# wenbowen123/catgrasp

Hardware: NVIDIA H100
Metric: candidate grasps scored/sec (higher is better)
Workload: dtype f32 (128->1024 layer f16 x f16 single pass on wgmma, f32 accumulate; other layers bf16 hi/lo x3)

## Files before the change

### catgrasp_b200/csrc/cg_tc_ptx.cuh

```cuda
#pragma once
#include <cuda_bf16.h>
#include <cuda_fp16.h>
#include <stdint.h>

namespace cg_ptx {

__device__ __forceinline__ uint32_t smem_u32(const void *p) { return static_cast<uint32_t>(__cvta_generic_to_shared(p)); }
__device__ __forceinline__ void mbar_init(uint32_t bar, uint32_t count) {
  asm volatile("mbarrier.init.shared::cta.b64 [%0], %1;" ::"r"(bar), "r"(count));
}
__device__ __forceinline__ void mbar_init_fence() { asm volatile("fence.mbarrier_init.release.cluster;" ::: "memory"); }
__device__ __forceinline__ void mbar_expect_tx(uint32_t bar, uint32_t bytes) {
  asm volatile("mbarrier.arrive.expect_tx.shared::cta.b64 _, [%0], %1;" ::"r"(bar), "r"(bytes) : "memory");
}
__device__ __forceinline__ void mbar_arrive(uint32_t bar) {
  asm volatile("mbarrier.arrive.shared::cta.b64 _, [%0];" ::"r"(bar) : "memory");
}
__device__ __forceinline__ void mbar_wait(uint32_t bar, uint32_t parity) {
  asm volatile(
      "{\n\t.reg .pred p;\n\t"
      "CG_MBAR_WAIT:\n\t"
      "mbarrier.try_wait.parity.shared::cta.b64 p, [%0], %1;\n\t"
      "@!p bra CG_MBAR_WAIT;\n\t}"
      ::"r"(bar), "r"(parity)
      : "memory");
}
__device__ __forceinline__ void bulk_g2s(uint32_t dst, const void *src, uint32_t bytes, uint32_t bar) {
  asm volatile("cp.async.bulk.shared::cluster.global.mbarrier::complete_tx::bytes [%0], [%1], %2, [%3];" ::"r"(dst),
               "l"(src), "r"(bytes), "r"(bar)
               : "memory");
}
__device__ __forceinline__ void fence_proxy_async() { asm volatile("fence.proxy.async.shared::cta;" ::: "memory"); }

__device__ __forceinline__ uint64_t wg_desc(uint32_t saddr) {
  return (uint64_t)((saddr >> 4) & 0x3FFFu) | (1ull << 16) | ((uint64_t)(1024 >> 4) << 32) | (1ull << 62);
}
__device__ __forceinline__ void wg_fence() { asm volatile("wgmma.fence.sync.aligned;" ::: "memory"); }
__device__ __forceinline__ void wg_commit() { asm volatile("wgmma.commit_group.sync.aligned;" ::: "memory"); }
template <int N>
__device__ __forceinline__ void wg_wait() {
  asm volatile("wgmma.wait_group.sync.aligned %0;" ::"n"(N) : "memory");
}
template <int N>
__device__ __forceinline__ void wg_fence_regs(float *r) {
#pragma unroll
  for (int i = 0; i < N; i++) asm volatile("" : "+f"(r[i])::"memory");
}
template <int N>
__device__ __forceinline__ void wg_fence_regs(uint32_t *r) {
#pragma unroll
  for (int i = 0; i < N; i++) asm volatile("" : "+r"(r[i])::"memory");
}

#define CG_WG_D8(i) "+f"(d[i]), "+f"(d[i + 1]), "+f"(d[i + 2]), "+f"(d[i + 3]), "+f"(d[i + 4]), "+f"(d[i + 5]), \
                    "+f"(d[i + 6]), "+f"(d[i + 7])

template <bool F16>
__device__ __forceinline__ void wg_m64n64(float *d, const uint32_t *a, uint64_t bdesc, uint32_t accumulate) {
  if (F16) {
    asm volatile(
        "{\n\t.reg .pred p;\n\t"
        "setp.ne.b32 p, %37, 0;\n\t"
        "wgmma.mma_async.sync.aligned.m64n64k16.f32.f16.f16 "
        "{%0, %1, %2, %3, %4, %5, %6, %7, %8, %9, %10, %11, %12, %13, %14, %15, "
        "%16, %17, %18, %19, %20, %21, %22, %23, %24, %25, %26, %27, %28, %29, %30, %31}, "
        "{%32, %33, %34, %35}, %36, p, 1, 1, 0;\n\t}"
        : CG_WG_D8(0), CG_WG_D8(8), CG_WG_D8(16), CG_WG_D8(24)
        : "r"(a[0]), "r"(a[1]), "r"(a[2]), "r"(a[3]), "l"(bdesc), "r"(accumulate)
        : "memory");
  } else {
    asm volatile(
        "{\n\t.reg .pred p;\n\t"
        "setp.ne.b32 p, %37, 0;\n\t"
        "wgmma.mma_async.sync.aligned.m64n64k16.f32.bf16.bf16 "
        "{%0, %1, %2, %3, %4, %5, %6, %7, %8, %9, %10, %11, %12, %13, %14, %15, "
        "%16, %17, %18, %19, %20, %21, %22, %23, %24, %25, %26, %27, %28, %29, %30, %31}, "
        "{%32, %33, %34, %35}, %36, p, 1, 1, 0;\n\t}"
        : CG_WG_D8(0), CG_WG_D8(8), CG_WG_D8(16), CG_WG_D8(24)
        : "r"(a[0]), "r"(a[1]), "r"(a[2]), "r"(a[3]), "l"(bdesc), "r"(accumulate)
        : "memory");
  }
}

template <bool F16>
__device__ __forceinline__ void wg_m64n128(float *d, const uint32_t *a, uint64_t bdesc, uint32_t accumulate) {
  if (F16) {
    asm volatile(
        "{\n\t.reg .pred p;\n\t"
        "setp.ne.b32 p, %69, 0;\n\t"
        "wgmma.mma_async.sync.aligned.m64n128k16.f32.f16.f16 "
        "{%0, %1, %2, %3, %4, %5, %6, %7, %8, %9, %10, %11, %12, %13, %14, %15, "
        "%16, %17, %18, %19, %20, %21, %22, %23, %24, %25, %26, %27, %28, %29, %30, %31, "
        "%32, %33, %34, %35, %36, %37, %38, %39, %40, %41, %42, %43, %44, %45, %46, %47, "
        "%48, %49, %50, %51, %52, %53, %54, %55, %56, %57, %58, %59, %60, %61, %62, %63}, "
        "{%64, %65, %66, %67}, %68, p, 1, 1, 0;\n\t}"
        : CG_WG_D8(0), CG_WG_D8(8), CG_WG_D8(16), CG_WG_D8(24), CG_WG_D8(32), CG_WG_D8(40), CG_WG_D8(48), CG_WG_D8(56)
        : "r"(a[0]), "r"(a[1]), "r"(a[2]), "r"(a[3]), "l"(bdesc), "r"(accumulate)
        : "memory");
  } else {
    asm volatile(
        "{\n\t.reg .pred p;\n\t"
        "setp.ne.b32 p, %69, 0;\n\t"
        "wgmma.mma_async.sync.aligned.m64n128k16.f32.bf16.bf16 "
        "{%0, %1, %2, %3, %4, %5, %6, %7, %8, %9, %10, %11, %12, %13, %14, %15, "
        "%16, %17, %18, %19, %20, %21, %22, %23, %24, %25, %26, %27, %28, %29, %30, %31, "
        "%32, %33, %34, %35, %36, %37, %38, %39, %40, %41, %42, %43, %44, %45, %46, %47, "
        "%48, %49, %50, %51, %52, %53, %54, %55, %56, %57, %58, %59, %60, %61, %62, %63}, "
        "{%64, %65, %66, %67}, %68, p, 1, 1, 0;\n\t}"
        : CG_WG_D8(0), CG_WG_D8(8), CG_WG_D8(16), CG_WG_D8(24), CG_WG_D8(32), CG_WG_D8(40), CG_WG_D8(48), CG_WG_D8(56)
        : "r"(a[0]), "r"(a[1]), "r"(a[2]), "r"(a[3]), "l"(bdesc), "r"(accumulate)
        : "memory");
  }
}
#undef CG_WG_D8

__device__ __forceinline__ void split_bf16x2(float x0, float x1, uint32_t &h, uint32_t &l) {
  const __nv_bfloat162 hh = __floats2bfloat162_rn(x0, x1);
  h = *reinterpret_cast<const uint32_t *>(&hh);
  const __nv_bfloat162 ll = __floats2bfloat162_rn(x0 - __uint_as_float(h << 16), x1 - __uint_as_float(h & 0xffff0000u));
  l = *reinterpret_cast<const uint32_t *>(&ll);
}
__device__ __forceinline__ void split_f16x2(float x0, float x1, uint32_t &h, uint32_t &l) {
  x0 = fminf(fmaxf(x0, -65504.f), 65504.f);
  x1 = fminf(fmaxf(x1, -65504.f), 65504.f);
  const __half2 hh = __floats2half2_rn(x0, x1);
  const float2 hf = __half22float2(hh);
  const __half2 ll = __floats2half2_rn(x0 - hf.x, x1 - hf.y);
  h = *reinterpret_cast<const uint32_t *>(&hh);
  l = *reinterpret_cast<const uint32_t *>(&ll);
}

template <int KS, bool F16>
__device__ __forceinline__ void d_to_a(const float *d, uint32_t (*hi)[4], uint32_t (*lo)[4]) {
#pragma unroll
  for (int j = 0; j < KS; j++)
#pragma unroll
    for (int r = 0; r < 4; r++) {
      if (F16) split_f16x2(d[8 * j + 2 * r], d[8 * j + 2 * r + 1], hi[j][r], lo[j][r]);
      else split_bf16x2(d[8 * j + 2 * r], d[8 * j + 2 * r + 1], hi[j][r], lo[j][r]);
    }
}

__host__ __device__ __forceinline__ uint32_t row_chunk_off(int row, int c16) {
  return (uint32_t)(row >> 3) * 1024u + (uint32_t)(row & 7) * 128u + (uint32_t)((c16 ^ (row & 7)) << 4);
}

}
```

### catgrasp_b200/csrc/cg_trunk_tc.cu

```cuda
#include <limits.h>
#include <stdlib.h>

#include <algorithm>

#include "cg_tc_ptx.cuh"
#include "cg_trunk_common.cuh"

namespace {
using namespace cg_trunk;
using namespace cg_ptx;

constexpr int NCW = 8;
constexpr int PROD_WARP = NCW;
constexpr int HELP_WARP = NCW + 1;
constexpr int NHELP = 3 * 32;
constexpr int NTC = (NCW + 4) * 32;
constexpr int NCHUNK = 8;
constexpr uint32_t PIECE = 16384;
constexpr uint32_t W1_OFF = 0;
constexpr uint32_t W2_OFF = PIECE;
constexpr uint32_t RING_OFF = 3 * PIECE;
constexpr uint32_t RING_BYTES = 8 * PIECE;
constexpr uint32_t SACC_OFF = RING_OFF + RING_BYTES;
constexpr uint32_t SACC_BYTES = 2 * 2 * NCHUNK * 4 * 32 * 8;
constexpr uint32_t KEYS_OFF = SACC_OFF + SACC_BYTES;
constexpr uint32_t KEYS_BYTES = 2 * 1024 * 4;
constexpr uint32_t MISC_OFF = KEYS_OFF + KEYS_BYTES;
constexpr int NSLOT_MAX = 8;
constexpr uint32_t IMG_W3B = NCHUNK * 2 * 2 * PIECE;
constexpr uint32_t IMG_W2 = 2 * PIECE, IMG_W1 = PIECE;
constexpr uint32_t IMG_W2_OFF = IMG_W3B, IMG_W1_OFF = IMG_W3B + IMG_W2;
constexpr uint32_t IMG_W3H_OFF = IMG_W1_OFF + IMG_W1;
constexpr uint32_t IMG_W3H = NCHUNK * 2 * PIECE;

struct Misc {
  float w0[6 * 64];
  float bias0[64];
  float bias1[64];
  float bias2[128];
  double pinv[12];
  double mean[6];
  double sden[6];
  float T3[12];
  unsigned long long full_bar[NSLOT_MAX];
  unsigned long long empty_bar[NSLOT_MAX];
  unsigned long long w_bar;
  unsigned long long cand_bar;
  unsigned long long front_bar;
  unsigned long long keys_bar[2];
};

constexpr size_t SMEM_BYTES = MISC_OFF + sizeof(Misc);
static_assert(SMEM_BYTES <= 232448, "exceeds the 227 KB per-CTA shared memory of sm_90");

template <int STEP>
__device__ __forceinline__ void max_butterfly_step(float *x, int lane) {
  const bool up = (lane & STEP) != 0;
#pragma unroll
  for (int k = 0; k < STEP / 2; k++) {
    const float send = up ? x[k] : x[k + STEP / 2];
    const float keep = up ? x[k + STEP / 2] : x[k];
    x[k] = fmaxf(keep, __shfl_xor_sync(0xffffffffu, send, STEP));
  }
}

#ifdef CG_EXPERIMENTS
enum { TL_START, TL_INPUT, TL_FRONT, TL_L3, TL_L3_WAIT, TL_RING, TL_NPHASE };
constexpr int TL_CTAS = 8, TL_REC = 8;
__host__ __device__ constexpr int TL_STRIDE(int B) { return B >= TL_CTAS ? B / TL_CTAS : 1; }
#define TL_PARAM , unsigned long long *tl
#define TL_ARG(p) , p
#else
#define TL_PARAM
#define TL_ARG(p)
#endif

template <int PASSES>
__global__ void __launch_bounds__(NTC, 1) trunk_tc_kernel(const cg_trunk_args a TL_PARAM) {
  constexpr int NSLOT = PASSES == 3 ? 4 : 8;
  constexpr uint32_t SLOT_BYTES = PASSES == 3 ? 2 * PIECE : PIECE;
  constexpr bool F16 = PASSES < 3;
  extern __shared__ __align__(1024) unsigned char smem[];
  if ((smem_u32(smem) & 1023u) != 0u) __trap();
  Misc &S = *reinterpret_cast<Misc *>(smem + MISC_OFF);
  float2 *sacc = reinterpret_cast<float2 *>(smem + SACC_OFF);
  uint32_t *keys = reinterpret_cast<uint32_t *>(smem + KEYS_OFF);
  const int tid = threadIdx.x, warp = __shfl_sync(0xffffffffu, tid >> 5, 0), lane = tid & 31;
  const int N = a.N;
  const int ntiles = (N + TP - 1) / TP;
  const long long T = (long long)a.B * ntiles;
  const int t_begin = (int)(blockIdx.x * T / gridDim.x);
  const int my_tiles = (int)((blockIdx.x + 1) * T / gridDim.x) - t_begin;
  const int b_first = t_begin / ntiles;
  const int ncand = (t_begin + my_tiles - 1) / ntiles - b_first + 1;
  const unsigned char *img = static_cast<const unsigned char *>(a.tc_img);
  const bool has_l1 = a.stage1_mode != 0;
  const uint32_t smem_s = smem_u32(smem);
  const uint32_t w1_s = smem_s + W1_OFF, w2_s = smem_s + W2_OFF, ring_s = smem_s + RING_OFF;
  const uint32_t misc_s = smem_s + MISC_OFF;
  const uint32_t full_s = misc_s + (uint32_t)offsetof(Misc, full_bar), empty_s = misc_s + (uint32_t)offsetof(Misc, empty_bar);
  const uint32_t wbar_s = misc_s + (uint32_t)offsetof(Misc, w_bar);
  const uint32_t cand_s = misc_s + (uint32_t)offsetof(Misc, cand_bar), front_s = misc_s + (uint32_t)offsetof(Misc, front_bar);
  const uint32_t keys_s = misc_s + (uint32_t)offsetof(Misc, keys_bar);

  for (int i = tid; i < 6 * 64; i += NTC) S.w0[i] = a.l0.Wt[i];
  if (tid < 64) {
    S.bias0[tid] = a.l0.b[tid];
    S.bias1[tid] = (a.stage1_mode == 1) ? a.l1.b[tid] : 0.f;
  }
  if (tid < 128) S.bias2[tid] = a.l2.b[tid];
  if (a.in.x_direct == nullptr && tid < 6) {
    S.mean[tid] = a.in.mean ? a.in.mean[tid] : 0.0;
    S.sden[tid] = a.in.stdv ? 1.0 / (a.in.stdv[tid] + 1e-15) : 1.0;
  }
  for (int i = tid; i < (int)(SACC_BYTES / 8); i += NTC) sacc[i] = make_float2(-INFINITY, -INFINITY);
  for (int i = tid; i < 2 * 1024; i += NTC) keys[i] = 0u;
  if (tid == 0) {
    for (int i = 0; i < NSLOT; i++) {
      mbar_init(full_s + 8u * i, 1);
      mbar_init(empty_s + 8u * i, NCW);
    }
    mbar_init(wbar_s, 1);
    mbar_init(cand_s, NHELP);
    mbar_init(front_s, NCW * 32);
    mbar_init(keys_s, NCW * 32);
    mbar_init(keys_s + 8u, NCW * 32);
    mbar_init_fence();
  }
  __syncthreads();

  if (warp == PROD_WARP) {
    if (lane == 0) {
      mbar_expect_tx(wbar_s, IMG_W2 + (a.stage1_mode == 1 ? IMG_W1 : 0u));
      bulk_g2s(w2_s, img + IMG_W2_OFF, IMG_W2, wbar_s);
      if (a.stage1_mode == 1) bulk_g2s(w1_s, img + IMG_W1_OFF, IMG_W1, wbar_s);
      const unsigned char *w3src = img + (PASSES == 3 ? 0u : IMG_W3H_OFF);
      const int total = my_tiles * NCHUNK * 2;
      for (int gs = 0; gs < total; gs++) {
        const int s = gs % NSLOT;
        mbar_wait(empty_s + 8u * s, (((uint32_t)(gs / NSLOT)) & 1u) ^ 1u);
        mbar_expect_tx(full_s + 8u * s, SLOT_BYTES);
        bulk_g2s(ring_s + (uint32_t)s * SLOT_BYTES, w3src + (size_t)(gs % (NCHUNK * 2)) * SLOT_BYTES, SLOT_BYTES,
                 full_s + 8u * s);
      }
    }
    return;
  }

  if (warp >= HELP_WARP) {
    const int ht = tid - HELP_WARP * 32;
    for (int k = 0; k <= ncand; k++) {
      if (k < ncand) {
        const int b = b_first + k;
        constexpr int TU = (64 * 8 + NHELP - 1) / NHELP;
        uint32_t t64h[TU][4], t64l[TU][4];
        if (a.stage1_mode == 2) {
          const float *Tb = a.T64 + (size_t)b * 4096;
#pragma unroll
          for (int i = 0; i < TU; i++) {
            const int u = ht + NHELP * i;
            if (u < 512) {
              float v[8];
#pragma unroll
              for (int e = 0; e < 8; e++) v[e] = __ldg(Tb + (8 * (u >> 6) + e) * 64 + (u & 63));
#pragma unroll
              for (int e = 0; e < 4; e++) split_bf16x2(v[2 * e], v[2 * e + 1], t64h[i][e], t64l[i][e]);
            }
          }
        }
        double pinv[12];
        const bool do_pinv = a.in.x_direct == nullptr && ht == 0;
        if (do_pinv) pose_inverse(a.in.poses + (size_t)b * 16, pinv);
        const float t3 = (a.T3 && ht < 9) ? a.T3[b * 9 + ht] : 0.f;
        if (k > 0) mbar_wait(front_s, (uint32_t)(k - 1) & 1u);
        if (a.stage1_mode == 2) {
#pragma unroll
          for (int i = 0; i < TU; i++) {
            const int u = ht + NHELP * i;
            if (u < 512) {
              const uint32_t off = row_chunk_off(u & 63, u >> 6);
              *reinterpret_cast<uint4 *>(smem + W1_OFF + off) =
                  make_uint4(t64h[i][0], t64h[i][1], t64h[i][2], t64h[i][3]);
              *reinterpret_cast<uint4 *>(smem + W1_OFF + 8192 + off) =
                  make_uint4(t64l[i][0], t64l[i][1], t64l[i][2], t64l[i][3]);
            }
          }
          fence_proxy_async();
        }
        if (do_pinv) {
#pragma unroll
          for (int i = 0; i < 12; i++) S.pinv[i] = pinv[i];
        }
        if (ht < 9) S.T3[ht] = t3;
        mbar_arrive(cand_s);
      }
      if (k > 0) {
        const int kp = k - 1;
        mbar_wait(keys_s + 8u * (kp & 1), ((uint32_t)kp >> 1) & 1u);
        uint32_t *kb = keys + (kp & 1) * 1024;
        uint32_t *g = a.gmax_keys + (size_t)(b_first + kp) * 1024;
        for (int ch = ht; ch < 1024; ch += NHELP) {
          float m = cg_key2f(kb[ch]) + __ldg(&a.l3.b[ch]);
          if (a.relu3) m = fmaxf(m, 0.f);
          atomicMax(&g[ch], cg_f2key(m));
          kb[ch] = 0u;
        }
      }
    }
    return;
  }

  const int wg = warp >> 2, w4 = warp & 3, g = lane >> 2, q = lane & 3;
  float vmax = 0.f;
#ifdef CG_EXPERIMENTS
  const bool tl_on = tl != nullptr && blockIdx.x % TL_STRIDE(gridDim.x) == 0 &&
                     (int)(blockIdx.x / TL_STRIDE(gridDim.x)) < TL_CTAS;
  unsigned long long tl_sum[TL_NPHASE] = {}, tl_t0 = clock64(), tl_t = tl_t0, tl_s;
#define TL_MARK(phase)                   \
  do {                                   \
    const unsigned long long _t = clock64(); \
    tl_sum[phase] += _t - tl_t;          \
    tl_t = _t;                           \
  } while (0)
#define TL_SPAN_BEGIN() (tl_s = clock64())
#define TL_SPAN_END(phase) (tl_sum[phase] += clock64() - tl_s)
#else
#define TL_MARK(phase) ((void)0)
#define TL_SPAN_BEGIN() ((void)0)
#define TL_SPAN_END(phase) ((void)0)
#endif
  mbar_wait(wbar_s, 0u);

  auto fetch_id = [&](int b, int n) -> int {
    if (n >= N) n = N - 1;
    return (a.in.x_direct == nullptr && a.in.ids) ? __ldg(a.in.ids + (size_t)b * N + n) : n;
  };
  auto fetch_row = [&](int b, int id, double *r) {
    if (a.in.x_direct) {
      const float *xr = a.in.x_direct + ((size_t)b * N + id) * 6;
#pragma unroll
      for (int k = 0; k < 6; k++) r[k] = __ldg(xr + k);
    } else {
      const double *px = a.in.cloud_xyz + (size_t)id * 3;
      const double *pn = a.in.cloud_nrm + (size_t)id * 3;
#pragma unroll
      for (int k = 0; k < 3; k++) {
        r[k] = __ldg(px + k);
        r[3 + k] = __ldg(pn + k);
      }
    }
  };
  auto finish_row = [&](const double *r, float *v) {
    if (a.in.x_direct) {
#pragma unroll
      for (int k = 0; k < 6; k++) v[k] = (float)r[k];
    } else {
      const double x = r[0], y = r[1], z = r[2];
      const double nx = r[3], ny = r[4], nz = r[5];
      const double *R = S.pinv;
      double w[6];
      w[0] = R[0] * x + R[1] * y + R[2] * z + R[9];
      w[1] = R[3] * x + R[4] * y + R[5] * z + R[10];
      w[2] = R[6] * x + R[7] * y + R[8] * z + R[11];
      w[3] = R[0] * nx + R[1] * ny + R[2] * nz;
      w[4] = R[3] * nx + R[4] * ny + R[5] * nz;
      w[5] = R[6] * nx + R[7] * ny + R[8] * nz;
#pragma unroll
      for (int k = 0; k < 6; k++) v[k] = (float)((w[k] - S.mean[k]) * S.sden[k]);
    }
    if (a.T3) {
      const float x = v[0], y = v[1], z = v[2];
      v[0] = fmaf(z, S.T3[6], fmaf(y, S.T3[3], x * S.T3[0]));
      v[1] = fmaf(z, S.T3[7], fmaf(y, S.T3[4], x * S.T3[1]));
      v[2] = fmaf(z, S.T3[8], fmaf(y, S.T3[5], x * S.T3[2]));
    }
  };

  uint32_t gslot = 0;
  auto slot_of = [&](int c, int kb) { return (gslot + 2u * c + kb) % NSLOT; };
  auto phase_of = [&](int c, int kb) { return ((gslot + 2u * c + kb) / NSLOT) & 1u; };

  const int prow = wg * 64 + w4 * 16 + g;
  constexpr int L3_GROUP = PASSES == 1 ? 8 : 4;
  constexpr bool ROW_PREFETCH = PASSES == 1;
  double r0[6], r1[6];
  int id0, id1;
  {
    const int j = t_begin - b_first * ntiles;
    id0 = fetch_id(b_first, j * TP + prow);
    id1 = fetch_id(b_first, j * TP + prow + 8);
    if (ROW_PREFETCH) {
      fetch_row(b_first, id0, r0);
      fetch_row(b_first, id1, r1);
    }
  }
  if (wg == 1) asm volatile("bar.sync 2, 256;" ::: "memory");
  TL_MARK(TL_START);
  for (int it = 0; it < my_tiles; it++) {
    const int b = (t_begin + it) / ntiles, j = t_begin + it - b * ntiles, ci = b - b_first;
    const bool cand_first = it == 0 || j == 0, cand_last = it + 1 == my_tiles || j + 1 == ntiles;
    const int p0 = j * TP + prow;
    if (cand_first) mbar_wait(cand_s, (uint32_t)ci & 1u);
    float d64[32];
    {
      float v0[6], v1[6];
      if (!ROW_PREFETCH) {
        fetch_row(b, id0, r0);
        fetch_row(b, id1, r1);
      }
      finish_row(r0, v0);
      finish_row(r1, v1);
      TL_MARK(TL_INPUT);
#pragma unroll
      for (int m = 0; m < 8; m++)
#pragma unroll
        for (int e = 0; e < 2; e++) {
          const int c = 8 * m + 2 * q + e;
          float o0 = S.bias0[c], o1 = o0;
#pragma unroll
          for (int k = 0; k < 6; k++) {
            const float w = S.w0[k * 64 + c];
            o0 = fmaf(v0[k], w, o0);
            o1 = fmaf(v1[k], w, o1);
          }
          d64[4 * m + e] = fmaxf(o0, 0.f);
          d64[4 * m + 2 + e] = fmaxf(o1, 0.f);
        }
    }
    uint32_t xh[8][4], xl[8][4];
    if (has_l1) {
      d_to_a<4, false>(d64, xh, xl);
      wg_fence_regs<16>(xh[0]);
      wg_fence_regs<16>(xl[0]);
      wg_fence_regs<32>(d64);
      wg_fence();
#pragma unroll
      for (int ks = 0; ks < 4; ks++) {
        const uint64_t bh = wg_desc(w1_s + 32u * ks), bl = wg_desc(w1_s + 8192u + 32u * ks);
        wg_m64n64<false>(d64, xl[ks], bh, ks > 0 ? 1u : 0u);
        wg_m64n64<false>(d64, xh[ks], bl, 1u);
        wg_m64n64<false>(d64, xh[ks], bh, 1u);
      }
      wg_commit();
      wg_wait<0>();
      wg_fence_regs<32>(d64);
      wg_fence_regs<16>(xh[0]);
      wg_fence_regs<16>(xl[0]);
#pragma unroll
      for (int i = 0; i < 32; i++) {
        if (a.stage1_mode == 1) d64[i] = fmaxf(d64[i] + S.bias1[8 * (i >> 2) + 2 * q + (i & 1)], 0.f);
      }
      if (a.pf_out) {
#pragma unroll
        for (int r = 0; r < 2; r++) {
          const int n = p0 + 8 * r;
          if (n < N) {
            float *dst = a.pf_out + ((size_t)b * N + n) * 64 + 2 * q;
#pragma unroll
            for (int m = 0; m < 8; m++)
              *reinterpret_cast<float2 *>(dst + 8 * m) = make_float2(d64[4 * m + 2 * r], d64[4 * m + 2 * r + 1]);
          }
        }
      }
    }
    if (cand_last) mbar_arrive(front_s);
    float acc[64];
    d_to_a<4, false>(d64, xh, xl);
    wg_fence_regs<16>(xh[0]);
    wg_fence_regs<16>(xl[0]);
    wg_fence_regs<64>(acc);
    wg_fence();
#pragma unroll
    for (int ks = 0; ks < 4; ks++) {
      const uint64_t bh = wg_desc(w2_s + 32u * ks), bl = wg_desc(w2_s + PIECE + 32u * ks);
      wg_m64n128<false>(acc, xl[ks], bh, ks > 0 ? 1u : 0u);
      wg_m64n128<false>(acc, xh[ks], bl, 1u);
      wg_m64n128<false>(acc, xh[ks], bh, 1u);
    }
    wg_commit();
    wg_wait<0>();
    wg_fence_regs<64>(acc);
    wg_fence_regs<16>(xh[0]);
    wg_fence_regs<16>(xl[0]);
    if (it == 0 && wg == 0) asm volatile("bar.arrive 2, 256;" ::: "memory");
    TL_MARK(TL_FRONT);
#pragma unroll
    for (int i = 0; i < 64; i++) acc[i] = fmaxf(acc[i] + S.bias2[8 * (i >> 2) + 2 * q + (i & 1)], 0.f);
    if (PASSES == 1) {
#pragma unroll
      for (int j = 0; j < 8; j++)
#pragma unroll
        for (int r = 0; r < 4; r++) {
          const float x0 = acc[8 * j + 2 * r], x1 = acc[8 * j + 2 * r + 1];
          vmax = fmaxf(vmax, fmaxf(x0, x1));
          asm("cvt.rn.satfinite.f16x2.f32 %0, %1, %2;" : "=r"(xh[j][r]) : "f"(x1), "f"(x0));
        }
    } else {
      if (PASSES == 2) {
#pragma unroll
        for (int i = 0; i < 64; i++) vmax = fmaxf(vmax, acc[i]);
      }
      d_to_a<8, F16>(acc, xh, xl);
    }
    wg_fence_regs<32>(xh[0]);
    if (PASSES != 1) wg_fence_regs<32>(xl[0]);
    auto issue = [&](int h, float *d) {
      const int c = h >> 1;
      if ((h & 1) == 0) {
        TL_SPAN_BEGIN();
        mbar_wait(full_s + 8u * slot_of(c, 0), phase_of(c, 0));
        mbar_wait(full_s + 8u * slot_of(c, 1), phase_of(c, 1));
        TL_SPAN_END(TL_RING);
      }
      wg_fence_regs<32>(d);
      wg_fence();
#pragma unroll
      for (int kb = 0; kb < 2; kb++) {
        const uint32_t ws = ring_s + slot_of(c, kb) * SLOT_BYTES + (uint32_t)(h & 1) * (PIECE / 2);
#pragma unroll
        for (int ks = 0; ks < 4; ks++) {
          const int j = kb * 4 + ks;
          const uint32_t first = (kb | ks) ? 1u : 0u;
          const uint64_t bw = wg_desc(ws + 32u * ks);
          if (PASSES == 3) {
            const uint64_t bl = wg_desc(ws + PIECE + 32u * ks);
            wg_m64n64<false>(d, xl[j], bw, first);
            wg_m64n64<false>(d, xh[j], bl, 1u);
            wg_m64n64<false>(d, xh[j], bw, 1u);
          } else if (PASSES == 2) {
            wg_m64n64<true>(d, xl[j], bw, first);
            wg_m64n64<true>(d, xh[j], bw, 1u);
          } else {
            wg_m64n64<true>(d, xh[j], bw, first);
          }
        }
      }
      wg_commit();
      wg_fence_regs<32>(d);
    };
    auto reduce = [&](int h, const float *d) {
      const int c = h >> 1;
      if (h & 1) {
        __syncwarp();
        if (lane == 0) {
          mbar_arrive(empty_s + 8u * slot_of(c, 0));
          mbar_arrive(empty_s + 8u * slot_of(c, 1));
        }
      }
      float x[16];
#pragma unroll
      for (int i = 0; i < 8; i++) {
        x[2 * i] = fmaxf(d[4 * i], d[4 * i + 2]);
        x[2 * i + 1] = fmaxf(d[4 * i + 1], d[4 * i + 3]);
      }
      max_butterfly_step<16>(x, lane);
      max_butterfly_step<8>(x, lane);
      max_butterfly_step<4>(x, lane);
      float2 &slot = sacc[((wg * 2 * NCHUNK + h) * 4 + w4) * 32 + lane];
      const float2 old = slot;
      slot = make_float2(fmaxf(old.x, x[0]), fmaxf(old.y, x[1]));
    };
    const int nt = t_begin + it + (it + 1 < my_tiles ? 1 : 0);
    const int nb = nt / ntiles, pn = (nt - nb * ntiles) * TP + prow;
    id0 = fetch_id(nb, pn);
    id1 = fetch_id(nb, pn + 8);
#pragma unroll 1
    for (int h0 = 0; h0 < 2 * NCHUNK; h0 += L3_GROUP) {
      if (ROW_PREFETCH && h0 == L3_GROUP) {
        fetch_row(nb, id0, r0);
        fetch_row(nb, id1, r1);
      }
      float acc3[2][32];
      issue(h0, acc3[0]);
#pragma unroll
      for (int j = 0; j < L3_GROUP; j++) {
        if (j + 1 < L3_GROUP) issue(h0 + j + 1, acc3[(j + 1) & 1]);
        TL_SPAN_BEGIN();
        if (j + 1 < L3_GROUP) wg_wait<1>();
        else wg_wait<0>();
        TL_SPAN_END(TL_L3_WAIT);
        wg_fence_regs<32>(acc3[j & 1]);
        reduce(h0 + j, acc3[j & 1]);
      }
    }
    wg_fence_regs<32>(xh[0]);
    if (PASSES != 1) wg_fence_regs<32>(xl[0]);
    gslot += 2u * NCHUNK;
    if (cand_last) {
      uint32_t *kk = keys + (ci & 1) * 1024;
#pragma unroll 4
      for (int h = 0; h < 2 * NCHUNK; h++) {
        float2 &slot = sacc[((wg * 2 * NCHUNK + h) * 4 + w4) * 32 + lane];
        const float2 v = slot;
        atomicMax(&kk[64 * h + 2 * lane], cg_f2key(v.x));
        atomicMax(&kk[64 * h + 2 * lane + 1], cg_f2key(v.y));
        slot = make_float2(-INFINITY, -INFINITY);
      }
      mbar_arrive(keys_s + 8u * (ci & 1));
    }
    TL_MARK(TL_L3);
  }
  if (F16 && vmax > 65504.f && a.ovf_flag) atomicOr(a.ovf_flag, 1u);
#ifdef CG_EXPERIMENTS
  if (tl_on && lane == 0) {
    unsigned long long *o = tl + ((size_t)(blockIdx.x / TL_STRIDE(gridDim.x)) * NCW + warp) * TL_REC;
#pragma unroll
    for (int p = 0; p < TL_NPHASE; p++) o[p] = tl_sum[p];
    o[TL_NPHASE] = (unsigned long long)my_tiles;
    o[TL_NPHASE + 1] = clock64() - tl_t0;
  }
#endif
#undef TL_MARK
#undef TL_SPAN_BEGIN
#undef TL_SPAN_END
}

}

size_t cg_tc_image_bytes() { return (size_t)IMG_W3H_OFF + IMG_W3H; }

int cg_tc_prepare(cg_ctx *ctx, const float *Wt3, const float *Wt2, const float *Wt1, void *dst_dev, int *f16_ok) {
  CG_CUDA(ctx, cudaFuncSetAttribute(trunk_tc_kernel<3>, cudaFuncAttributeMaxDynamicSharedMemorySize, (int)SMEM_BYTES));
  CG_CUDA(ctx, cudaFuncSetAttribute(trunk_tc_kernel<2>, cudaFuncAttributeMaxDynamicSharedMemorySize, (int)SMEM_BYTES));
  CG_CUDA(ctx, cudaFuncSetAttribute(trunk_tc_kernel<1>, cudaFuncAttributeMaxDynamicSharedMemorySize, (int)SMEM_BYTES));
  float wmax = 0.f;
  for (size_t i = 0; i < (size_t)128 * 1024; i++) wmax = fmaxf(wmax, fabsf(Wt3[i]));
  *f16_ok = (wmax < 65504.f) ? 1 : 0;
  std::vector<unsigned char> img(cg_tc_image_bytes(), 0);
  for (int ch = 0; ch < NCHUNK; ch++)
    for (int kb = 0; kb < 2; kb++) {
      unsigned char *hi = img.data() + (size_t)(ch * 2 + kb) * 2 * PIECE;
      cg_pack_bf16x2_block(Wt3, 1024, ch * 128, 128, kb * 64, hi, hi + PIECE);
    }
  cg_pack_bf16x2_block(Wt2, 128, 0, 128, 0, img.data() + IMG_W2_OFF, img.data() + IMG_W2_OFF + PIECE);
  if (Wt1) cg_pack_bf16x2_block(Wt1, 64, 0, 64, 0, img.data() + IMG_W1_OFF, img.data() + IMG_W1_OFF + 8192);
  for (int ch = 0; ch < NCHUNK; ch++)
    for (int r = 0; r < 128; r++)
      for (int k = 0; k < 128; k++) {
        const __half h = __float2half_rn(Wt3[(size_t)k * 1024 + ch * 128 + r]);
        unsigned short bits;
        memcpy(&bits, &h, 2);
        const size_t off = (size_t)IMG_W3H_OFF + (size_t)(ch * 2 + (k >> 6)) * PIECE + row_chunk_off(r, (k & 63) >> 3) +
                           (size_t)(k & 7) * 2;
        memcpy(img.data() + off, &bits, 2);
      }
  CG_CUDA(ctx, cudaMemcpyAsync(dst_dev, img.data(), img.size(), cudaMemcpyHostToDevice, ctx->stream));
  CG_CUDA(ctx, cudaStreamSynchronize(ctx->stream));
  return CG_OK;
}

int cg_trunk_launch_tc(cg_ctx *ctx, const cg_trunk_args &a) {
  CG_REQUIRE(ctx, a.B > 0 && a.N > 0, "trunk: B,N must be positive");
  CG_REQUIRE(ctx, a.tc_img != nullptr, "trunk: tensor-core weight image missing");
  const long long tiles = (long long)a.B * ((a.N + TP - 1) / TP);
  CG_REQUIRE(ctx, tiles <= INT_MAX, "trunk: too many tiles in one launch");
  const int grid = (int)std::min<long long>(ctx->num_sms, tiles);
  const int passes = !a.tc_f16_ok || ctx->engine == 1 ? 3 : (ctx->engine == 2 ? 2 : 1);
#ifdef CG_EXPERIMENTS
  static const bool timeline = getenv("CG_TRUNK_TIMELINE") && atoi(getenv("CG_TRUNK_TIMELINE")) != 0;
  unsigned long long *tl = nullptr;
  const size_t tl_words = (size_t)TL_CTAS * NCW * TL_REC;
  if (timeline) {
    CG_CUDA(ctx, cudaMallocAsync(&tl, tl_words * 8, ctx->stream));
    CG_CUDA(ctx, cudaMemsetAsync(tl, 0, tl_words * 8, ctx->stream));
  }
#endif
  if (passes == 3) trunk_tc_kernel<3><<<grid, NTC, SMEM_BYTES, ctx->stream>>>(a TL_ARG(tl));
  else if (passes == 2) trunk_tc_kernel<2><<<grid, NTC, SMEM_BYTES, ctx->stream>>>(a TL_ARG(tl));
  else trunk_tc_kernel<1><<<grid, NTC, SMEM_BYTES, ctx->stream>>>(a TL_ARG(tl));
  CG_LAUNCH_CHECK(ctx);
#ifdef CG_EXPERIMENTS
  if (timeline) {
    std::vector<unsigned long long> h(tl_words);
    CG_CUDA(ctx, cudaMemcpyAsync(h.data(), tl, tl_words * 8, cudaMemcpyDeviceToHost, ctx->stream));
    CG_CUDA(ctx, cudaFreeAsync(tl, ctx->stream));
    CG_CUDA(ctx, cudaStreamSynchronize(ctx->stream));
    double sum[TL_NPHASE + 1] = {}, tiles = 0;
    int recs = 0;
    for (int r = 0; r < TL_CTAS * NCW; r++) {
      const unsigned long long *o = &h[(size_t)r * TL_REC];
      if (o[TL_NPHASE] == 0) continue;
      for (int p = 0; p < TL_NPHASE; p++) sum[p] += (double)o[p];
      sum[TL_NPHASE] += (double)o[TL_NPHASE + 1];
      tiles += (double)o[TL_NPHASE];
      recs++;
    }
    if (recs > 0) {
      const double l3 = 128.0 * 128 * 1024 / 2048 * passes, l12 = 128.0 * 64 * (128 + (a.stage1_mode ? 64 : 0)) * 3 / 2048;
      const double tot = sum[TL_NPHASE] / tiles;
      fprintf(stderr,
              "[trunk-timeline] passes=%d B=%d N=%d stage1=%d tiles/CTA=%.0f warps=%d  clk/tile: start %.0f  input %.0f  "
              "front %.0f  l3 %.0f (wgmma-wait %.0f, ring-wait %.0f)  total %.0f  | tensor work %.0f clk/tile -> "
              "busy %.1f%%\n",
              passes, a.B, a.N, a.stage1_mode, tiles / recs, recs, sum[TL_START] / tiles, sum[TL_INPUT] / tiles,
              sum[TL_FRONT] / tiles, sum[TL_L3] / tiles, sum[TL_L3_WAIT] / tiles, sum[TL_RING] / tiles, tot, l3 + l12,
              100.0 * (l3 + l12) / tot);
    }
  }
#endif
  return CG_OK;
}
```

Baseline: 366,500.

## Widen layer-3 wgmma to n128, rebalance registers, double-buffer per-candidate constants

In single-pass f16 mode the 128->1024 layer now issues m64n128 wgmma tiles instead of pairs of n64, which halves the instruction count and the per-group reduction overhead. The max-butterfly and shared accumulator layout become float4 per chunk to match. Producer and helper warps lower their register budget with setmaxnreg while consumer warps raise theirs. Helpers now write pose-inverse and T3 into double-buffered shared slots before waiting, so they no longer stage them in registers, and row fetches are interleaved into the layer-3 loop. The costs are more live accumulator registers per tile, which may cause spills, and a changed slot and phase scheme that assumes each tile's ring usage is even.

Result: faster. 385,000 (median of 6 runs) (+5.1%).

```diff
diff --git a/catgrasp_b200/csrc/cg_tc_ptx.cuh b/catgrasp_b200/csrc/cg_tc_ptx.cuh
--- a/catgrasp_b200/csrc/cg_tc_ptx.cuh
+++ b/catgrasp_b200/csrc/cg_tc_ptx.cuh
@@ -114,6 +114,22 @@
 }
 #undef CG_WG_D8
 
+template <int N, bool F16>
+__device__ __forceinline__ void wg_m64nN(float *d, const uint32_t *a, uint64_t bdesc, uint32_t accumulate) {
+  static_assert(N == 64 || N == 128, "wgmma tile width");
+  if constexpr (N == 128) wg_m64n128<F16>(d, a, bdesc, accumulate);
+  else wg_m64n64<F16>(d, a, bdesc, accumulate);
+}
+
+template <int R>
+__device__ __forceinline__ void setmaxnreg_dec() {
+  asm volatile("setmaxnreg.dec.sync.aligned.u32 %0;" ::"n"(R));
+}
+template <int R>
+__device__ __forceinline__ void setmaxnreg_inc() {
+  asm volatile("setmaxnreg.inc.sync.aligned.u32 %0;" ::"n"(R));
+}
+
 __device__ __forceinline__ void split_bf16x2(float x0, float x1, uint32_t &h, uint32_t &l) {
   const __nv_bfloat162 hh = __floats2bfloat162_rn(x0, x1);
   h = *reinterpret_cast<const uint32_t *>(&hh);
diff --git a/catgrasp_b200/csrc/cg_trunk_tc.cu b/catgrasp_b200/csrc/cg_trunk_tc.cu
--- a/catgrasp_b200/csrc/cg_trunk_tc.cu
+++ b/catgrasp_b200/csrc/cg_trunk_tc.cu
@@ -15,6 +15,11 @@
 constexpr int HELP_WARP = NCW + 1;
 constexpr int NHELP = 3 * 32;
 constexpr int NTC = (NCW + 4) * 32;
+template <int PASSES>
+constexpr int R_CONS = PASSES == 1 ? 216 : 200;
+template <int PASSES>
+constexpr int R_PROD = (168 * NTC - 256 * R_CONS<PASSES>) / 128 / 8 * 8;
+static_assert(R_PROD<1> == 72 && R_PROD<3> == 104 && R_CONS<1> % 8 == 0 && R_CONS<3> % 8 == 0, "register pool");
 constexpr int NCHUNK = 8;
 constexpr uint32_t PIECE = 16384;
 constexpr uint32_t W1_OFF = 0;
@@ -22,7 +27,7 @@
 constexpr uint32_t RING_OFF = 3 * PIECE;
 constexpr uint32_t RING_BYTES = 8 * PIECE;
 constexpr uint32_t SACC_OFF = RING_OFF + RING_BYTES;
-constexpr uint32_t SACC_BYTES = 2 * 2 * NCHUNK * 4 * 32 * 8;
+constexpr uint32_t SACC_BYTES = 2 * NCHUNK * 4 * 32 * 16;
 constexpr uint32_t KEYS_OFF = SACC_OFF + SACC_BYTES;
 constexpr uint32_t KEYS_BYTES = 2 * 1024 * 4;
 constexpr uint32_t MISC_OFF = KEYS_OFF + KEYS_BYTES;
@@ -38,10 +43,10 @@
   float bias0[64];
   float bias1[64];
   float bias2[128];
-  double pinv[12];
+  double pinv[2][12];
   double mean[6];
   double sden[6];
-  float T3[12];
+  float T3[2][12];
   unsigned long long full_bar[NSLOT_MAX];
   unsigned long long empty_bar[NSLOT_MAX];
   unsigned long long w_bar;
@@ -53,13 +58,13 @@
 constexpr size_t SMEM_BYTES = MISC_OFF + sizeof(Misc);
 static_assert(SMEM_BYTES <= 232448, "exceeds the 227 KB per-CTA shared memory of sm_90");
 
-template <int STEP>
+template <int STEP, int KEEP>
 __device__ __forceinline__ void max_butterfly_step(float *x, int lane) {
   const bool up = (lane & STEP) != 0;
 #pragma unroll
-  for (int k = 0; k < STEP / 2; k++) {
-    const float send = up ? x[k] : x[k + STEP / 2];
-    const float keep = up ? x[k + STEP / 2] : x[k];
+  for (int k = 0; k < KEEP; k++) {
+    const float send = up ? x[k] : x[k + KEEP];
+    const float keep = up ? x[k + KEEP] : x[k];
     x[k] = fmaxf(keep, __shfl_xor_sync(0xffffffffu, send, STEP));
   }
 }
@@ -83,16 +88,23 @@
   extern __shared__ __align__(1024) unsigned char smem[];
   if ((smem_u32(smem) & 1023u) != 0u) __trap();
   Misc &S = *reinterpret_cast<Misc *>(smem + MISC_OFF);
-  float2 *sacc = reinterpret_cast<float2 *>(smem + SACC_OFF);
+  float4 *sacc = reinterpret_cast<float4 *>(smem + SACC_OFF);
   uint32_t *keys = reinterpret_cast<uint32_t *>(smem + KEYS_OFF);
   const int tid = threadIdx.x, warp = __shfl_sync(0xffffffffu, tid >> 5, 0), lane = tid & 31;
   const int N = a.N;
   const int ntiles = (N + TP - 1) / TP;
-  const long long T = (long long)a.B * ntiles;
-  const int t_begin = (int)(blockIdx.x * T / gridDim.x);
-  const int my_tiles = (int)((blockIdx.x + 1) * T / gridDim.x) - t_begin;
-  const int b_first = t_begin / ntiles;
-  const int ncand = (t_begin + my_tiles - 1) / ntiles - b_first + 1;
+  struct Range {
+    int t_begin, my_tiles, b_first, ncand;
+  };
+  auto tile_range = [&]() {
+    const long long T = (long long)a.B * ntiles;
+    Range r;
+    r.t_begin = (int)(blockIdx.x * T / gridDim.x);
+    r.my_tiles = (int)((blockIdx.x + 1) * T / gridDim.x) - r.t_begin;
+    r.b_first = r.t_begin / ntiles;
+    r.ncand = (r.t_begin + r.my_tiles - 1) / ntiles - r.b_first + 1;
+    return r;
+  };
   const unsigned char *img = static_cast<const unsigned char *>(a.tc_img);
   const bool has_l1 = a.stage1_mode != 0;
   const uint32_t smem_s = smem_u32(smem);
@@ -113,7 +125,8 @@
     S.mean[tid] = a.in.mean ? a.in.mean[tid] : 0.0;
     S.sden[tid] = a.in.stdv ? 1.0 / (a.in.stdv[tid] + 1e-15) : 1.0;
   }
-  for (int i = tid; i < (int)(SACC_BYTES / 8); i += NTC) sacc[i] = make_float2(-INFINITY, -INFINITY);
+  for (int i = tid; i < (int)(SACC_BYTES / 16); i += NTC)
+    sacc[i] = make_float4(-INFINITY, -INFINITY, -INFINITY, -INFINITY);
   for (int i = tid; i < 2 * 1024; i += NTC) keys[i] = 0u;
   if (tid == 0) {
     for (int i = 0; i < NSLOT; i++) {
@@ -129,69 +142,56 @@
   }
   __syncthreads();
 
-  if (warp == PROD_WARP) {
-    if (lane == 0) {
-      mbar_expect_tx(wbar_s, IMG_W2 + (a.stage1_mode == 1 ? IMG_W1 : 0u));
-      bulk_g2s(w2_s, img + IMG_W2_OFF, IMG_W2, wbar_s);
-      if (a.stage1_mode == 1) bulk_g2s(w1_s, img + IMG_W1_OFF, IMG_W1, wbar_s);
-      const unsigned char *w3src = img + (PASSES == 3 ? 0u : IMG_W3H_OFF);
-      const int total = my_tiles * NCHUNK * 2;
-      for (int gs = 0; gs < total; gs++) {
-        const int s = gs % NSLOT;
-        mbar_wait(empty_s + 8u * s, (((uint32_t)(gs / NSLOT)) & 1u) ^ 1u);
-        mbar_expect_tx(full_s + 8u * s, SLOT_BYTES);
-        bulk_g2s(ring_s + (uint32_t)s * SLOT_BYTES, w3src + (size_t)(gs % (NCHUNK * 2)) * SLOT_BYTES, SLOT_BYTES,
-                 full_s + 8u * s);
-      }
-    }
-    return;
-  }
-
-  if (warp >= HELP_WARP) {
+  if (warp >= PROD_WARP) {
+    setmaxnreg_dec<R_PROD<PASSES>>();
+    const Range rg = tile_range();
+    if (warp == PROD_WARP) {
+      if (lane == 0) {
+        mbar_expect_tx(wbar_s, IMG_W2 + (a.stage1_mode == 1 ? IMG_W1 : 0u));
+        bulk_g2s(w2_s, img + IMG_W2_OFF, IMG_W2, wbar_s);
+        if (a.stage1_mode == 1) bulk_g2s(w1_s, img + IMG_W1_OFF, IMG_W1, wbar_s);
+        const unsigned char *w3src = img + (PASSES == 3 ? 0u : IMG_W3H_OFF);
+        const int total = rg.my_tiles * NCHUNK * 2;
+        for (int gs = 0; gs < total; gs++) {
+          const int s = gs % NSLOT;
+          mbar_wait(empty_s + 8u * s, (((uint32_t)(gs / NSLOT)) & 1u) ^ 1u);
+          mbar_expect_tx(full_s + 8u * s, SLOT_BYTES);
+          bulk_g2s(ring_s + (uint32_t)s * SLOT_BYTES, w3src + (size_t)(gs % (NCHUNK * 2)) * SLOT_BYTES, SLOT_BYTES,
+                   full_s + 8u * s);
+        }
+      }
+      return;
+    }
+
     const int ht = tid - HELP_WARP * 32;
+    const int b_first = rg.b_first, ncand = rg.ncand;
     for (int k = 0; k <= ncand; k++) {
       if (k < ncand) {
         const int b = b_first + k;
-        constexpr int TU = (64 * 8 + NHELP - 1) / NHELP;
-        uint32_t t64h[TU][4], t64l[TU][4];
+        if (a.in.x_direct == nullptr && ht == 0) pose_inverse(a.in.poses + (size_t)b * 16, S.pinv[k & 1]);
+        if (ht < 9) S.T3[k & 1][ht] = a.T3 ? a.T3[b * 9 + ht] : 0.f;
+        if (k > 0) mbar_wait(front_s, (uint32_t)(k - 1) & 1u);
         if (a.stage1_mode == 2) {
+          constexpr int TU = (64 * 8 + NHELP - 1) / NHELP;
           const float *Tb = a.T64 + (size_t)b * 4096;
 #pragma unroll
           for (int i = 0; i < TU; i++) {
             const int u = ht + NHELP * i;
             if (u < 512) {
+              const float *src = Tb + (u >> 6) * 512 + (u & 63);
               float v[8];
-#pragma unroll
-              for (int e = 0; e < 8; e++) v[e] = __ldg(Tb + (8 * (u >> 6) + e) * 64 + (u & 63));
-#pragma unroll
-              for (int e = 0; e < 4; e++) split_bf16x2(v[2 * e], v[2 * e + 1], t64h[i][e], t64l[i][e]);
-            }
-          }
-        }
-        double pinv[12];
-        const bool do_pinv = a.in.x_direct == nullptr && ht == 0;
-        if (do_pinv) pose_inverse(a.in.poses + (size_t)b * 16, pinv);
-        const float t3 = (a.T3 && ht < 9) ? a.T3[b * 9 + ht] : 0.f;
-        if (k > 0) mbar_wait(front_s, (uint32_t)(k - 1) & 1u);
-        if (a.stage1_mode == 2) {
-#pragma unroll
-          for (int i = 0; i < TU; i++) {
-            const int u = ht + NHELP * i;
-            if (u < 512) {
+              uint32_t hi[4], lo[4];
+#pragma unroll
+              for (int e = 0; e < 8; e++) v[e] = __ldg(src + e * 64);
+#pragma unroll
+              for (int e = 0; e < 4; e++) split_bf16x2(v[2 * e], v[2 * e + 1], hi[e], lo[e]);
               const uint32_t off = row_chunk_off(u & 63, u >> 6);
-              *reinterpret_cast<uint4 *>(smem + W1_OFF + off) =
-                  make_uint4(t64h[i][0], t64h[i][1], t64h[i][2], t64h[i][3]);
-              *reinterpret_cast<uint4 *>(smem + W1_OFF + 8192 + off) =
-                  make_uint4(t64l[i][0], t64l[i][1], t64l[i][2], t64l[i][3]);
+              *reinterpret_cast<uint4 *>(smem + W1_OFF + off) = make_uint4(hi[0], hi[1], hi[2], hi[3]);
+              *reinterpret_cast<uint4 *>(smem + W1_OFF + 8192 + off) = make_uint4(lo[0], lo[1], lo[2], lo[3]);
             }
           }
           fence_proxy_async();
         }
-        if (do_pinv) {
-#pragma unroll
-          for (int i = 0; i < 12; i++) S.pinv[i] = pinv[i];
-        }
-        if (ht < 9) S.T3[ht] = t3;
         mbar_arrive(cand_s);
       }
       if (k > 0) {
@@ -210,6 +210,9 @@
     return;
   }
 
+  setmaxnreg_inc<R_CONS<PASSES>>();
+  const Range rg = tile_range();
+  const int t_begin = rg.t_begin, my_tiles = rg.my_tiles, b_first = rg.b_first;
   const int wg = warp >> 2, w4 = warp & 3, g = lane >> 2, q = lane & 3;
   float vmax = 0.f;
 #ifdef CG_EXPERIMENTS
@@ -250,14 +253,14 @@
       }
     }
   };
-  auto finish_row = [&](const double *r, float *v) {
+  auto finish_row = [&](const double *r, float *v, int par) {
     if (a.in.x_direct) {
 #pragma unroll
       for (int k = 0; k < 6; k++) v[k] = (float)r[k];
     } else {
       const double x = r[0], y = r[1], z = r[2];
       const double nx = r[3], ny = r[4], nz = r[5];
-      const double *R = S.pinv;
+      const double *R = S.pinv[par];
       double w[6];
       w[0] = R[0] * x + R[1] * y + R[2] * z + R[9];
       w[1] = R[3] * x + R[4] * y + R[5] * z + R[10];
@@ -269,30 +272,29 @@
       for (int k = 0; k < 6; k++) v[k] = (float)((w[k] - S.mean[k]) * S.sden[k]);
     }
     if (a.T3) {
+      const float *T3 = S.T3[par];
       const float x = v[0], y = v[1], z = v[2];
-      v[0] = fmaf(z, S.T3[6], fmaf(y, S.T3[3], x * S.T3[0]));
-      v[1] = fmaf(z, S.T3[7], fmaf(y, S.T3[4], x * S.T3[1]));
-      v[2] = fmaf(z, S.T3[8], fmaf(y, S.T3[5], x * S.T3[2]));
+      v[0] = fmaf(z, T3[6], fmaf(y, T3[3], x * T3[0]));
+      v[1] = fmaf(z, T3[7], fmaf(y, T3[4], x * T3[1]));
+      v[2] = fmaf(z, T3[8], fmaf(y, T3[5], x * T3[2]));
     }
   };
 
-  uint32_t gslot = 0;
-  auto slot_of = [&](int c, int kb) { return (gslot + 2u * c + kb) % NSLOT; };
-  auto phase_of = [&](int c, int kb) { return ((gslot + 2u * c + kb) / NSLOT) & 1u; };
+  static_assert(2 * NCHUNK % (2 * NSLOT) == 0, "a tile must pass every W3 slot an even number of times");
+  auto slot_of = [](int c, int kb) { return (uint32_t)(2 * c + kb) % NSLOT; };
+  auto phase_of = [](int c, int kb) { return (uint32_t)((2 * c + kb) / NSLOT) & 1u; };
 
   const int prow = wg * 64 + w4 * 16 + g;
-  constexpr int L3_GROUP = PASSES == 1 ? 8 : 4;
-  constexpr bool ROW_PREFETCH = PASSES == 1;
+  constexpr int L3N = PASSES == 1 ? 128 : 64;
+  constexpr int L3_GROUP = PASSES == 1 ? 1024 / L3N : 8;
   double r0[6], r1[6];
   int id0, id1;
   {
     const int j = t_begin - b_first * ntiles;
     id0 = fetch_id(b_first, j * TP + prow);
     id1 = fetch_id(b_first, j * TP + prow + 8);
-    if (ROW_PREFETCH) {
-      fetch_row(b_first, id0, r0);
-      fetch_row(b_first, id1, r1);
-    }
+    fetch_row(b_first, id0, r0);
+    fetch_row(b_first, id1, r1);
   }
   if (wg == 1) asm volatile("bar.sync 2, 256;" ::: "memory");
   TL_MARK(TL_START);
@@ -304,12 +306,8 @@
     float d64[32];
     {
       float v0[6], v1[6];
-      if (!ROW_PREFETCH) {
-        fetch_row(b, id0, r0);
-        fetch_row(b, id1, r1);
-      }
-      finish_row(r0, v0);
-      finish_row(r1, v1);
+      finish_row(r0, v0, ci & 1);
+      finish_row(r1, v1, ci & 1);
       TL_MARK(TL_INPUT);
 #pragma unroll
       for (int m = 0; m < 8; m++)
@@ -404,19 +402,23 @@
     }
     wg_fence_regs<32>(xh[0]);
     if (PASSES != 1) wg_fence_regs<32>(xl[0]);
+    if (F16) wg_fence_regs<1>(&vmax);
+    constexpr int NG = 1024 / L3N, GPC = 128 / L3N;
     auto issue = [&](int h, float *d) {
-      const int c = h >> 1;
-      if ((h & 1) == 0) {
+      const int c = h / GPC;
+      if (h % GPC == 0) {
         TL_SPAN_BEGIN();
         mbar_wait(full_s + 8u * slot_of(c, 0), phase_of(c, 0));
         mbar_wait(full_s + 8u * slot_of(c, 1), phase_of(c, 1));
         TL_SPAN_END(TL_RING);
       }
-      wg_fence_regs<32>(d);
+      wg_fence_regs<L3N / 2>(d);
+      uint32_t ring = ring_s;
+      asm volatile("" : "+r"(ring));
       wg_fence();
 #pragma unroll
       for (int kb = 0; kb < 2; kb++) {
-        const uint32_t ws = ring_s + slot_of(c, kb) * SLOT_BYTES + (uint32_t)(h & 1) * (PIECE / 2);
+        const uint32_t ws = ring + slot_of(c, kb) * SLOT_BYTES + (uint32_t)(h % GPC) * (L3N * 128u);
 #pragma unroll
         for (int ks = 0; ks < 4; ks++) {
           const int j = kb * 4 + ks;
@@ -424,77 +426,90 @@
           const uint64_t bw = wg_desc(ws + 32u * ks);
           if (PASSES == 3) {
             const uint64_t bl = wg_desc(ws + PIECE + 32u * ks);
-            wg_m64n64<false>(d, xl[j], bw, first);
-            wg_m64n64<false>(d, xh[j], bl, 1u);
-            wg_m64n64<false>(d, xh[j], bw, 1u);
+            wg_m64nN<L3N, false>(d, xl[j], bw, first);
+            wg_m64nN<L3N, false>(d, xh[j], bl, 1u);
+            wg_m64nN<L3N, false>(d, xh[j], bw, 1u);
           } else if (PASSES == 2) {
-            wg_m64n64<true>(d, xl[j], bw, first);
-            wg_m64n64<true>(d, xh[j], bw, 1u);
+            wg_m64nN<L3N, true>(d, xl[j], bw, first);
+            wg_m64nN<L3N, true>(d, xh[j], bw, 1u);
           } else {
-            wg_m64n64<true>(d, xh[j], bw, first);
+            wg_m64nN<L3N, true>(d, xh[j], bw, first);
           }
         }
       }
       wg_commit();
-      wg_fence_regs<32>(d);
+      wg_fence_regs<L3N / 2>(d);
     };
     auto reduce = [&](int h, const float *d) {
-      const int c = h >> 1;
-      if (h & 1) {
+      const int c = h / GPC;
+      if (h % GPC == GPC - 1) {
         __syncwarp();
         if (lane == 0) {
           mbar_arrive(empty_s + 8u * slot_of(c, 0));
           mbar_arrive(empty_s + 8u * slot_of(c, 1));
         }
       }
-      float x[16];
-#pragma unroll
-      for (int i = 0; i < 8; i++) {
+      float x[L3N / 4];
+#pragma unroll
+      for (int i = 0; i < L3N / 8; i++) {
         x[2 * i] = fmaxf(d[4 * i], d[4 * i + 2]);
         x[2 * i + 1] = fmaxf(d[4 * i + 1], d[4 * i + 3]);
       }
-      max_butterfly_step<16>(x, lane);
-      max_butterfly_step<8>(x, lane);
-      max_butterfly_step<4>(x, lane);
-      float2 &slot = sacc[((wg * 2 * NCHUNK + h) * 4 + w4) * 32 + lane];
-      const float2 old = slot;
-      slot = make_float2(fmaxf(old.x, x[0]), fmaxf(old.y, x[1]));
+      max_butterfly_step<16, L3N / 8>(x, lane);
+      max_butterfly_step<8, L3N / 16>(x, lane);
+      max_butterfly_step<4, L3N / 32>(x, lane);
+      float4 &slot = sacc[((wg * NCHUNK + c) * 4 + w4) * 32 + lane];
+      if (L3N == 128) {
+        const float4 old = slot;
+        slot = make_float4(fmaxf(old.x, x[0]), fmaxf(old.y, x[1]), fmaxf(old.z, x[2]), fmaxf(old.w, x[3]));
+      } else {
+        float2 &half = reinterpret_cast<float2 *>(&slot)[h % GPC];
+        const float2 old = half;
+        half = make_float2(fmaxf(old.x, x[0]), fmaxf(old.y, x[1]));
+      }
     };
     const int nt = t_begin + it + (it + 1 < my_tiles ? 1 : 0);
     const int nb = nt / ntiles, pn = (nt - nb * ntiles) * TP + prow;
     id0 = fetch_id(nb, pn);
     id1 = fetch_id(nb, pn + 8);
 #pragma unroll 1
-    for (int h0 = 0; h0 < 2 * NCHUNK; h0 += L3_GROUP) {
-      if (ROW_PREFETCH && h0 == L3_GROUP) {
+    for (int h0 = 0; h0 < NG; h0 += L3_GROUP) {
+      if (L3_GROUP < NG && h0 == L3_GROUP) {
         fetch_row(nb, id0, r0);
         fetch_row(nb, id1, r1);
       }
-      float acc3[2][32];
+      float acc3[2][L3N / 2];
       issue(h0, acc3[0]);
 #pragma unroll
       for (int j = 0; j < L3_GROUP; j++) {
         if (j + 1 < L3_GROUP) issue(h0 + j + 1, acc3[(j + 1) & 1]);
+        if (L3_GROUP == NG && j == 1) {
+          fetch_row(nb, id0, r0);
+          fetch_row(nb, id1, r1);
+        }
         TL_SPAN_BEGIN();
         if (j + 1 < L3_GROUP) wg_wait<1>();
         else wg_wait<0>();
         TL_SPAN_END(TL_L3_WAIT);
-        wg_fence_regs<32>(acc3[j & 1]);
+        wg_fence_regs<L3N / 2>(acc3[j & 1]);
         reduce(h0 + j, acc3[j & 1]);
       }
     }
     wg_fence_regs<32>(xh[0]);
     if (PASSES != 1) wg_fence_regs<32>(xl[0]);
-    gslot += 2u * NCHUNK;
     if (cand_last) {
-      uint32_t *kk = keys + (ci & 1) * 1024;
-#pragma unroll 4
-      for (int h = 0; h < 2 * NCHUNK; h++) {
-        float2 &slot = sacc[((wg * 2 * NCHUNK + h) * 4 + w4) * 32 + lane];
-        const float2 v = slot;
-        atomicMax(&kk[64 * h + 2 * lane], cg_f2key(v.x));
-        atomicMax(&kk[64 * h + 2 * lane + 1], cg_f2key(v.y));
-        slot = make_float2(-INFINITY, -INFINITY);
+      constexpr int HI = L3N == 128 ? 8 : 64;
+      const int col = g * (L3N / 8) + 2 * q;
+      uint32_t *kk = keys + (ci & 1) * 1024 + col;
+#pragma unroll 2
+      for (int c = 0; c < NCHUNK; c++) {
+        float4 &slot = sacc[((wg * NCHUNK + c) * 4 + w4) * 32 + lane];
+        const float4 v = slot;
+        atomicMax(&kk[128 * c], cg_f2key(v.x));
+        atomicMax(&kk[128 * c + 1], cg_f2key(v.y));
+        atomicMax(&kk[128 * c + HI], cg_f2key(v.z));
+        atomicMax(&kk[128 * c + HI + 1], cg_f2key(v.w));
+        slot = make_float4(-INFINITY, -INFINITY, -INFINITY, -INFINITY);
       }
       mbar_arrive(keys_s + 8u * (ci & 1));
     }
```
